# FatimaSohailll/KLT-Feature-Tracker-Acceleration-GPUs

Hardware: AMD Instinct MI355X
Metric: frames/sec + pyramid Gpix/s @1080p 5000 feats, 1/2/4/8 MI355X (higher is better)
Workload: dtype f32; 1 GPU; 1920x1080, 5000 features, sequential KLTTrackFeatures pass + KLTStoreFeatureList per frame, 2361 frames per GPU (BASELINE config 3; config 5 at N>1); device-resident: frames in HBM before timing, features and table stay on the device (the API-inclusive figure is the `api` key); chunk=64, chunk_requested=64, resolution=1920x1080, features=5000, frames=2361, parallelism=single GPU, reduction=exact

## Files before the change

include/klt_hip.h:

```cpp
#ifndef KLT_HIP_H
#define KLT_HIP_H

#include <stddef.h>

#ifdef __cplusplus
extern "C" {
#endif

#define KLT_HIP_MAX_TAPS 71
#define KLT_HIP_MAX_LEVELS 8
#define KLT_HIP_MAX_SLOTS 4

#define KLT_HIP_EXACT 0
#define KLT_HIP_FAST 1

typedef struct {
  int width;
  float k[KLT_HIP_MAX_TAPS];
} klt_hip_taps;

typedef struct {
  int ncols, nrows;
  int nlevels;
  int subsampling;
// ... 43 lines not shown
void klt_hip_ctx_destroy(klt_hip_ctx *ctx);
int klt_hip_ctx_reset(klt_hip_ctx *ctx);
int klt_hip_ctx_device(klt_hip_ctx *ctx);
int klt_hip_current_device(void);
const char *klt_hip_last_error(klt_hip_ctx *ctx);
const char *klt_hip_track_kernel(klt_hip_ctx *ctx);
int klt_hip_set_stream(klt_hip_ctx *ctx, void *stream);
void *klt_hip_get_stream(klt_hip_ctx *ctx);
int klt_hip_sync(klt_hip_ctx *ctx);
int klt_hip_device_count(void);

int klt_hip_upload_frame(klt_hip_ctx *ctx, int buf, const unsigned char *host, int ncols,
                         int nrows);
int klt_hip_build_pyramid(klt_hip_ctx *ctx, int slot, const klt_hip_pyr_desc *desc,
                          const unsigned char *frame, long pitch, int buf);

#define KLT_HIP_FRAME_GRAY8 0
#define KLT_HIP_FRAME_RGB8 1
#define KLT_HIP_FRAME_BGR8 2
#define KLT_HIP_FRAME_RGBA8 3
#define KLT_HIP_FRAME_BGRA8 4
int klt_hip_frame_bpp(int format);
int klt_hip_set_frame_format(klt_hip_ctx *ctx, int format);
int klt_hip_get_frame_format(klt_hip_ctx *ctx);
int klt_hip_gray_host(int format, const unsigned char *src, long pitch, int ncols, int nrows,
                      unsigned char *dst, long dst_pitch);
int klt_hip_to_gray(klt_hip_ctx *ctx, int format, const unsigned char *dev_src, long pitch, long stride,
                    int nframes, int ncols, int nrows, unsigned char *dev_dst, long dst_pitch, long dst_stride);
int klt_hip_set_path(klt_hip_ctx *ctx, int force_generic);
int klt_hip_set_track_order(klt_hip_ctx *ctx, int input_order);
int klt_hip_set_track_impl(klt_hip_ctx *ctx, int impl);
int klt_hip_set_track_merge(klt_hip_ctx *ctx, int on);
int klt_hip_set_lazy_grad(klt_hip_ctx *ctx, int on);
#define KLT_HIP_FB_REJECTED (-6)
int klt_hip_set_fb(klt_hip_ctx *ctx, int on, float max_dist);
int klt_hip_get_fb(klt_hip_ctx *ctx, int *on, float *max_dist);
int klt_hip_set_fb_table(klt_hip_ctx *ctx, float *dev_err, long stride);
int klt_hip_set_predict(klt_hip_ctx *ctx, int on, float *dev_vx, float *dev_vy);
int klt_hip_get_predict(klt_hip_ctx *ctx, int *on, float **dev_vx, float **dev_vy);
int klt_hip_set_predict_table(klt_hip_ctx *ctx, float *dev_tab_vx, float *dev_tab_vy, long stride);
#define KLT_HIP_MASKED (-7)
#define KLT_HIP_MASK_SELECT 1
#define KLT_HIP_MASK_TRACK 2
int klt_hip_set_mask(klt_hip_ctx *ctx, const unsigned char *dev_mask, long pitch, int flags);
int klt_hip_get_mask(klt_hip_ctx *ctx, const unsigned char **dev_mask, long *pitch, int *flags);
int klt_hip_set_track_prio(klt_hip_ctx *ctx, int on);
int klt_hip_set_track_count(klt_hip_ctx *ctx, int on);
int klt_hip_get_track_count(klt_hip_ctx *ctx, unsigned long long *solves, unsigned long long *passes,
                            int reset);
int klt_hip_set_track_patch(klt_hip_ctx *ctx, int on);
int klt_hip_set_prof(klt_hip_ctx *ctx, void *dev);
int klt_hip_set_host_threads(klt_hip_ctx *ctx, int workers);
int klt_hip_get_host_threads(klt_hip_ctx *ctx);
int klt_hip_register_host(klt_hip_ctx *ctx, const void *ptr, size_t bytes);
int klt_hip_unregister_host(klt_hip_ctx *ctx, const void *ptr);
int klt_hip_set_bank_budget(klt_hip_ctx *ctx, size_t bytes);
size_t klt_hip_get_bank_budget(klt_hip_ctx *ctx);
int klt_hip_frames_chunk(klt_hip_ctx *ctx);
size_t klt_hip_ctx_footprint(klt_hip_ctx *ctx);
int klt_hip_set_frames_overlap(klt_hip_ctx *ctx, int overlap);
int klt_hip_set_frames_tail(klt_hip_ctx *ctx, int waves_left);
int klt_hip_tail_threshold(unsigned base, unsigned launched, unsigned waves_left, unsigned *threshold);
int klt_hip_set_wave_times(klt_hip_ctx *ctx, void *dev);
int klt_hip_order_slot(int n, int xcd_per, int n_live, int rank, int lost, int *slot);
int klt_hip_band_order_probe(klt_hip_ctx *ctx, const float *y, const int *val, int n, int nrows, int *perm_out);
int klt_hip_fused_path(klt_hip_ctx *ctx, const klt_hip_pyr_desc *desc);
// ... 134 lines not shown
```

klt-feature-tracker-acceleration-gpus_amd/csrc/klt_dev.h:

```cpp
#pragma once

#include <hip/hip_runtime.h>
#include <stdint.h>

#include <string>

#include "klt_hip.h"

namespace kltdev {

constexpr int kWave = 64;
constexpr int kBlock = 256;

constexpr int kTracked = 0, kNotFound = -1, kSmallDet = -2, kMaxIter = -3, kOOB = -4, kLargeResidue = -5;

__host__ __device__ __forceinline__ int clampi(int v, int lo, int hi) { return v < lo ? lo : (v > hi ? hi : v); }

struct RTaps {
  int w;
  float k[KLT_HIP_MAX_TAPS];
};

inline RTaps reverse_taps(const klt_hip_taps &t) {
  RTaps r;
// ... 127 lines not shown
  const float *ai, *agx, *agy;
  const float *bi, *bgx, *bgy;
  int aw, ah, bw, bh;
  const float *xp, *yp;
  const float *x, *y;
  int *v;
  float *xo, *yo;
  float *aff;
  int *state;
  float *store;
  int n;
  AffParams p;
};

struct TrkAffArgs {
  AffParams p;
  float *aff;
  int *state;
  float *store;
  int fresh;
  int lds_wave;
  float *tab_aff;
  int *tab_state;
  long stride;
};
#ifndef KLT_AFF_CH
#define KLT_AFF_CH 64
#endif
constexpr int kAffChunk = KLT_AFF_CH;

hipError_t launch_pyr_l0(hipStream_t st, const uint8_t *src, int pitch, long stride, int W, int H, const DefTaps &T,
                         int vec_u8, int vec_out, float *img, float *gx, float *gy, float *hs, int W1, int do_hs,
                         long fs0, long fsh, int F, int ty0, int ty1, int py0 = 0, int py1 = 1 << 30, int il = 0,
                         int fmt = KLT_HIP_FRAME_GRAY8);
hipError_t launch_pyr_l1(hipStream_t st, const float *hs, int W1, int H, int H1, const DefTaps &T, int vec,
                         float *img1, float *gx1, float *gy1, long fsh, long fs1, int F, int ty0, int ty1, int il = 0,
                         int thin = 0);
constexpr int kL1ThinRows = 8;
hipError_t launch_u8_to_f32(hipStream_t st, const uint8_t *src, long pitch, int W, int H, float *out);
hipError_t launch_px_to_f32(hipStream_t st, const uint8_t *src, long pitch, int W, int H, int fmt, float *out);
hipError_t launch_to_gray(hipStream_t st, int fmt, const uint8_t *src, long pitch, long stride, int n, int W, int H,
                          uint8_t *dst, long dpitch, long dstride);
hipError_t launch_rows(hipStream_t st, const float *in, int W, int H, const RTaps &t, float *out);
hipError_t launch_cols(hipStream_t st, const float *in, int W, int H, const RTaps &t, float *out);
hipError_t launch_subsample(hipStream_t st, const float *in, int W, int ss, float *out, int W1, int H1);
hipError_t launch_min_eigen(hipStream_t st, const float *gx, const float *gy, int W, int ps, int bx, int by, int step,
                            int nx, int ny, int hw, int hh, int *out, const char **name = nullptr);
struct GradTaps {
  float g[2 * kRG + 1], d[2 * kRG + 1];
};
hipError_t launch_min_eigen_img(hipStream_t st, const float *img, int W, int H, const GradTaps &t, int bx, int by,
                                int step, int nx, int ny, int *out, const char **name = nullptr);
hipError_t launch_min_eigen_multi(hipStream_t st, const float *rec, long frame_stride, const EigMultiArgs &m, int W,
                                  int bx, int by, int step, int nx, int ny, int *maps, const char **name = nullptr);
hipError_t launch_synth(hipStream_t st, unsigned long long seed, int t0, int n, int W, int H, int row0, uint8_t *out,
                        long pitch, long fstride);
hipError_t launch_selftest_sqrt(const double *in, double *out, int n);
hipError_t launch_from_il(hipStream_t st, const float *il, float *img, float *gx, float *gy, long n);
hipError_t launch_to_il(hipStream_t st, const float *plane, float *il, int field, long n);
hipError_t launch_copy_words(hipStream_t st, const void *src, void *dst, long n);
hipError_t launch_selftest_div(const float *a, const float *b, float *out, int n);
hipError_t launch_selftest_solve2(const float *in, float step, float min_det, float *out, int *ok, int n);

hipError_t launch_track_frames(hipStream_t st, bool exact, bool li, bool patch, bool win7, int npx,
                               const TrkArgs &a, const TrkFramesArgs &b, float *x, float *y, int *v, int n,
                               const TrkFbArgs *fb = nullptr, const TrkAffArgs *af = nullptr);
size_t track_affine_lds_bytes(int mode);
// ... 60 lines not shown
```

klt-feature-tracker-acceleration-gpus_amd/csrc/pyramid.hip:

```cpp
#pragma clang fp contract(off)

#include <math.h>
#include <stdlib.h>

#include "klt_dev.h"
#include "klt_synth.h"

namespace kltdev {
namespace {

typedef float f2 __attribute__((ext_vector_type(2)));

typedef float f4 __attribute__((ext_vector_type(4)));

__device__ __forceinline__ f4 ld4(const float *p) { return *reinterpret_cast<const f4 *>(p); }
static_assert(kHsSlab == 16, "hs slab width");
__device__ __forceinline__ unsigned hs_at32(int y, int X, int H) {
  return ((unsigned)(X >> 4) * (unsigned)H + (unsigned)y) * 16u + (unsigned)(X & 15);
}
__device__ __forceinline__ void st4(float *p, f4 v) { *reinterpret_cast<f4 *>(p) = v; }
__device__ __forceinline__ void st4_out(float *p, f4 v) { __builtin_nontemporal_store(v, reinterpret_cast<f4 *>(p)); }
__device__ __forceinline__ void st2_out(float *p, f2 v) { __builtin_nontemporal_store(v, reinterpret_cast<f2 *>(p)); }
typedef float f3u __attribute__((ext_vector_type(3), aligned(4)));
__device__ __forceinline__ void st3_out(float *p, f3u v) { __builtin_nontemporal_store(v, reinterpret_cast<f3u *>(p)); }
// ... 551 lines not shown
template <bool IL, int TH_, bool IMG, int FMT>
__global__ __launch_bounds__(L0G<TH_>::NT) void k_pyr_l0_px(const uint8_t *__restrict__ src, int spitch, int W, int H,
                                                      DefTaps T, int vec_u8, float *__restrict__ img0,
                                                      float *__restrict__ gx0, float *__restrict__ gy0,
                                                      float *__restrict__ hs, int hsW, int do_hs, int vec_out,
                                                      long fs_src, long fs0, long fs_hs, int ty0, int tiles_x,
                                                      int tiles_y, int py0, int py1) {
  static_assert(FMT != KLT_HIP_FRAME_GRAY8, "gray frames take k_pyr_l0");
  using G = L0G<TH_, IMG ? 0 : kRG>;
  __shared__ __attribute__((aligned(16))) float lds[G::LDS];
  int bx, by;
  if (!xcd_tile(tiles_x, tiles_y, bx, by)) return;
#ifdef KLT_PYR_PROF
  const int tid = threadIdx.x;
  PYR_STAMP(0)
#endif
  const int C0 = bx * G::TW, R0 = (by + ty0) * G::TH;
  src += blockIdx.z * fs_src;
  img0 += blockIdx.z * fs0;
  gx0 += blockIdx.z * fs0;
  gy0 += blockIdx.z * fs0;
  hs += blockIdx.z * fs_hs;
  const bool cols_in = C0 >= 12 && C0 + 84 <= W, rows_in = R0 >= 5 && R0 + G::TH + 7 <= H;
  const bool interior = vec_u8 && vec_out && (hsW * G::SS == W) && (hsW % 2 == 0) && cols_in && rows_in;
  const bool planes = by + ty0 >= py0 && by + ty0 < py1;
  if (interior)
    pyr_l0_tile<true, IL, TH_, IMG, FMT>(lds, src, spitch, W, H, T, vec_u8, img0, gx0, gy0, hs, hsW, do_hs, vec_out, C0,
                                         R0, threadIdx.x, planes, true, true);
  else
    pyr_l0_tile<false, IL, TH_, IMG, FMT>(lds, src, spitch, W, H, T, vec_u8, img0, gx0, gy0, hs, hsW, do_hs, vec_out, C0,
                                          R0, threadIdx.x, planes, cols_in, rows_in);
}

template <int TH_>
struct L1G {
  static constexpr int RG = kRG, RP = kRP, SS = kSS, TW = geom::L1_TW, TH = TH_, NT = 256;
  static constexpr int JW = 40;
  static constexpr int JH = TH + 2 * RG;
  static constexpr int HR = SS * (JH - 1) + 2 * RP + 1;
  static constexpr int LDS_H = HR * JW, LDS_J = JH * JW, LDS_X = JH * TW;
  static constexpr int LDS = LDS_H + LDS_J;
  static_assert(2 * LDS_X + TH * 3 * TW <= LDS_H, "tx/ty and the interleaved output tile reuse the hs region");
};
static_assert(L1G<geom::L1_TH>::HR == geom::L1_HR, "geometry");
constexpr int kL1ThinTH = 8;

template <bool IL, int TH_>
__global__ __launch_bounds__(256) void k_pyr_l1(const float *__restrict__ hs, int W1, int H, int H1,
                                                DefTaps T, int vec, float *__restrict__ img1,
                                                float *__restrict__ gx1, float *__restrict__ gy1,
                                                long fs_hs, long fs1, int ty0, int tiles_x, int tiles_y) {
  using G = L1G<TH_>;
  constexpr int RG = G::RG, RP = G::RP, SS = G::SS, TW = G::TW, TH = G::TH, NT = G::NT, JW = G::JW, JH = G::JH,
                HR = G::HR, LDS_H = G::LDS_H, LDS_X = G::LDS_X, LDS = G::LDS;
  hs += blockIdx.z * fs_hs;
  img1 += blockIdx.z * fs1;
  gx1 += blockIdx.z * fs1;
  gy1 += blockIdx.z * fs1;
  __shared__ __attribute__((aligned(16))) float lds[LDS];
  float *hl = lds;
  float *im = lds + LDS_H;
  float *tx = lds;
  float *ty = lds + LDS_X;
  float *stg = lds + 2 * LDS_X;

  int bx, by;
// ... 485 lines not shown
    const float acc = lane == kSumGxx   ? S[0]
                      : lane == kSumGxy ? S[1]
                      : lane == kSumGyy ? S[2]
                      : lane == kSumEx  ? S[3]
                      : lane == kSumEy  ? S[4]
                                        : __int_as_float(0x7fc00000 + lane);
    float dx = 0.0f, dy = 0.0f, d = 0.0f, du = 0.0f;
    const float det1 = solve_det(S[0], S[1], S[2]);
    const float det2 = solve_det(lane_of(acc, kSumGxx), lane_of(acc, kSumGxy), lane_of(acc, kSumGyy));
    const int k1 = !(det1 < min_det), k2 = !(det2 < min_det), k3 = k1;
    if (k1) solve1(S, step, det1, dx, dy);
    if (k2) d = solve2(acc, lane_of(acc, kSumGxy), step, det2);
    if (k3) du = solve2u(S, lane == 0, step, det1);
    const float r[6] = {dx, dy, lane_of(d, 0), lane_of(d, 1), lane_of(du, 0), lane_of(du, 1)};
    if (lane == 0) {
#pragma unroll
      for (int k = 0; k < 6; ++k) out[6 * (long)i + k] = r[k];
      ok[i] = k1 | (k2 << 1) | (k3 << 2);
    }
  }
}

}

constexpr int kL0WideMinRows = 2000;
bool l0_wide() {
  static const bool on = [] {
    const char *v = getenv("KLT_L0_WIDE");
    return !(v && *v && atoi(v) == 0);
  }();
  return on;
}

namespace {
template <int FMT>
hipError_t launch_pyr_l0_px(hipStream_t st, const uint8_t *src, int pitch, long stride, int W, int H, const DefTaps &T,
                            int vec_u8, int vec_out, float *img, float *gx, float *gy, float *hs, int W1, int do_hs,
                            long fs0, long fsh, int F, int ty0, int ty1, int py0, int py1, int il) {
  const int tx = (W + l0::TW - 1) / l0::TW;
  const int nty = (H + l0::G32::TH - 1) / l0::G32::TH;
  if (l0_wide() && H >= kL0WideMinRows && ty0 == 0 && ty1 == nty && py0 == 0 && py1 >= nty) {
    using G = L0G<64>;
    const int ty = (H + G::TH - 1) / G::TH;
    const dim3 grid(xcd_grid(tx * ty), 1, F);
    if (il == kLayoutImg)
      hipLaunchKernelGGL((k_pyr_l0_px<false, 64, true, FMT>), grid, dim3(G::NT), 0, st, src, pitch, W, H, T, vec_u8, img,
                         gx, gy, hs, W1, do_hs, vec_out, stride, fs0, fsh, 0, tx, ty, 0, ty);
    else if (il)
      hipLaunchKernelGGL((k_pyr_l0_px<true, 64, false, FMT>), grid, dim3(G::NT), 0, st, src, pitch, W, H, T, vec_u8, img,
                         gx, gy, hs, W1, do_hs, vec_out, stride, fs0, fsh, 0, tx, ty, 0, ty);
    else
      hipLaunchKernelGGL((k_pyr_l0_px<false, 64, false, FMT>), grid, dim3(G::NT), 0, st, src, pitch, W, H, T, vec_u8,
                         img, gx, gy, hs, W1, do_hs, vec_out, stride, fs0, fsh, 0, tx, ty, 0, ty);
    return hipGetLastError();
  }
  using G = l0::G32;
  const dim3 grid(xcd_grid(tx * (ty1 - ty0)), 1, F);
  if (il == kLayoutImg)
    hipLaunchKernelGGL((k_pyr_l0_px<false, 32, true, FMT>), grid, dim3(G::NT), 0, st, src, pitch, W, H, T, vec_u8, img,
                       gx, gy, hs, W1, do_hs, vec_out, stride, fs0, fsh, ty0, tx, ty1 - ty0, py0, py1);
  else if (il)
    hipLaunchKernelGGL((k_pyr_l0_px<true, 32, false, FMT>), grid, dim3(G::NT), 0, st, src, pitch, W, H, T, vec_u8, img,
                       gx, gy, hs, W1, do_hs, vec_out, stride, fs0, fsh, ty0, tx, ty1 - ty0, py0, py1);
  else
    hipLaunchKernelGGL((k_pyr_l0_px<false, 32, false, FMT>), grid, dim3(G::NT), 0, st, src, pitch, W, H, T, vec_u8, img,
                       gx, gy, hs, W1, do_hs, vec_out, stride, fs0, fsh, ty0, tx, ty1 - ty0, py0, py1);
  return hipGetLastError();
}
}

hipError_t launch_pyr_l0(hipStream_t st, const uint8_t *src, int pitch, long stride, int W, int H, const DefTaps &T,
                         int vec_u8, int vec_out, float *img, float *gx, float *gy, float *hs, int W1, int do_hs,
                         long fs0, long fsh, int F, int ty0, int ty1, int py0, int py1, int il, int fmt) {
  const int tx = (W + l0::TW - 1) / l0::TW;
  if (F <= 0 || ty1 <= ty0) return hipSuccess;
  switch (fmt) {
    case KLT_HIP_FRAME_GRAY8: break;
#define KLT_L0_PX(f)                                                                                               \
  case f:                                                                                                          \
    return launch_pyr_l0_px<f>(st, src, pitch, stride, W, H, T, vec_u8, vec_out, img, gx, gy, hs, W1, do_hs, fs0, \
                               fsh, F, ty0, ty1, py0, py1, il);
      KLT_L0_PX(KLT_HIP_FRAME_RGB8)
      KLT_L0_PX(KLT_HIP_FRAME_BGR8)
      KLT_L0_PX(KLT_HIP_FRAME_RGBA8)
      KLT_L0_PX(KLT_HIP_FRAME_BGRA8)
#undef KLT_L0_PX
    default: return hipErrorInvalidValue;
  }
#ifdef KLT_EXP_NOHS
  do_hs = 0;
#endif
  const int nty = (H + l0::G32::TH - 1) / l0::G32::TH;
  if (l0_wide() && H >= kL0WideMinRows && ty0 == 0 && ty1 == nty && py0 == 0 && py1 >= nty) {
    using G = L0G<64>;
    const int ty = (H + G::TH - 1) / G::TH;
    if (il == kLayoutImg)
      hipLaunchKernelGGL((k_pyr_l0<false, 64, true>), dim3(xcd_grid(tx * ty), 1, F), dim3(G::NT), 0, st, src, pitch, W,
                         H, T, vec_u8, img, gx, gy, hs, W1, do_hs, vec_out, stride, fs0, fsh, 0, tx, ty, 0, ty);
    else if (il)
      hipLaunchKernelGGL((k_pyr_l0<true, 64>), dim3(xcd_grid(tx * ty), 1, F), dim3(G::NT), 0, st, src, pitch, W, H, T,
                         vec_u8, img, gx, gy, hs, W1, do_hs, vec_out, stride, fs0, fsh, 0, tx, ty, 0, ty);
    else
      hipLaunchKernelGGL((k_pyr_l0<false, 64>), dim3(xcd_grid(tx * ty), 1, F), dim3(G::NT), 0, st, src, pitch, W, H,
                         T, vec_u8, img, gx, gy, hs, W1, do_hs, vec_out, stride, fs0, fsh, 0, tx, ty, 0, ty);
    return hipGetLastError();
  }
  using G = l0::G32;
  if (il == kLayoutImg)
    hipLaunchKernelGGL((k_pyr_l0<false, 32, true>), dim3(xcd_grid(tx * (ty1 - ty0)), 1, F), dim3(G::NT), 0, st, src,
                       pitch, W, H, T, vec_u8, img, gx, gy, hs, W1, do_hs, vec_out, stride, fs0, fsh, ty0, tx, ty1 - ty0,
                       py0, py1);
  else if (il)
    hipLaunchKernelGGL((k_pyr_l0<true, 32>), dim3(xcd_grid(tx * (ty1 - ty0)), 1, F), dim3(G::NT), 0, st, src, pitch, W,
                       H, T, vec_u8, img, gx, gy, hs, W1, do_hs, vec_out, stride, fs0, fsh, ty0, tx, ty1 - ty0, py0, py1);
  else
    hipLaunchKernelGGL((k_pyr_l0<false, 32>), dim3(xcd_grid(tx * (ty1 - ty0)), 1, F), dim3(G::NT), 0, st, src, pitch,
                       W, H, T, vec_u8, img, gx, gy, hs, W1, do_hs, vec_out, stride, fs0, fsh, ty0, tx, ty1 - ty0, py0,
                       py1);
  return hipGetLastError();
}

hipError_t launch_pyr_l1(hipStream_t st, const float *hs, int W1, int H, int H1, const DefTaps &T, int vec,
                         float *img1, float *gx1, float *gy1, long fsh, long fs1, int F, int ty0, int ty1, int il,
                         int thin) {
  const int tx = (W1 + geom::L1_TW - 1) / geom::L1_TW;
// ... 190 lines not shown
```

klt-feature-tracker-acceleration-gpus_amd/csrc/runtime.h:

```cpp
#pragma once

#include <sys/resource.h>
#include <math.h>
#include <stdarg.h>
#include <stdint.h>
#include <stdio.h>
#include <stdlib.h>
#include <string.h>

#include <algorithm>
#include <set>
#include <string>
#include <vector>

#include "host_pool.h"
#include "klt_dev.h"
#include "klt_hip.h"

#define KLT_API extern "C" __attribute__((visibility("default")))

#ifndef KLT_LAZY_GRAD_DEFAULT
#define KLT_LAZY_GRAD_DEFAULT 1
#endif

// ... 101 lines not shown
  bool caller_pending = false;
  Slot slot[KLT_HIP_MAX_SLOTS + 2];
  uint8_t *d_u8[2] = {nullptr, nullptr};
  uint8_t *h_u8[2] = {nullptr, nullptr};
  hipEvent_t u8_done[2] = {nullptr, nullptr};
  size_t u8_cap = 0;
  int u8_w[2] = {0, 0}, u8_h[2] = {0, 0};
  float *d_hs = nullptr;
  size_t hs_cap = 0;
  float *d_tmp[2] = {nullptr, nullptr};
  size_t tmp_cap[2] = {0, 0};
  float *d_fx = nullptr, *d_fy = nullptr;
  int *d_fv = nullptr;
  float *d_feat = nullptr, *h_feat = nullptr;
  int feat_mode = 2;
  size_t f_cap = 0;
  int *d_eig = nullptr;
  size_t eig_cap = 0;
  SelEngine *sel = nullptr;
  std::vector<std::pair<const unsigned char *, size_t>> registered;
  float *d_aff_store = nullptr;
  size_t aff_store_cap = 0;
  int aff_S = 0;
  float *d_aff = nullptr, *d_xp = nullptr, *d_yp = nullptr, *d_astage = nullptr;
  size_t aff_cap = 0, xp_cap = 0, yp_cap = 0, astage_cap = 0;
  int *d_astate = nullptr, *d_aidx = nullptr;
  size_t astate_cap = 0, aidx_cap = 0;
  std::string err;
  int force_generic = 0;
  int frame_format = KLT_HIP_FRAME_GRAY8;
  int track_order = 0;
  int track_patch = 1;
  int track_merge = 1;
  int lazy_grad = KLT_LAZY_GRAD_DEFAULT;
  RTaps lazy_gg, lazy_gd;
  int track_prio = 1;
  float *pl_scr[2][KLT_HIP_MAX_LEVELS] = {};
  size_t pl_cap[2][KLT_HIP_MAX_LEVELS] = {};
  int track_impl = 0;
  const char *track_kernel = nullptr;
  int fb_on = 0;
  float fb_dist = 0.0f;
  float *fb_tab = nullptr;
  long fb_stride = 0;
  int pred_on = 0;
  float *pred_vx = nullptr, *pred_vy = nullptr;
  float *pred_tvx = nullptr, *pred_tvy = nullptr;
  long pred_stride = 0;
  float *d_pred = nullptr;
  size_t pred_cap = 0;
  const unsigned char *mask = nullptr;
  long mask_pitch = 0;
  int mask_flags = 0;
  int aff_on = 0;
  AffParams aff_p{};
  float *aff_dev = nullptr;
  int *aff_state_dev = nullptr;
  float *aff_tab = nullptr;
  int *aff_stab = nullptr;
  long aff_tab_stride = 0;
  int aff_fresh = 1, aff_depth = 0;
  int rep_on = 0;
  klt_hip_replace_desc rep{};
  long rep_frames = 0, rep_runs = 0, rep_filled = 0;
  std::vector<unsigned char> rep_changed;
  int *d_rep_map = nullptr;
// ... 269 lines not shown
```

klt-feature-tracker-acceleration-gpus_amd/csrc/runtime.hip:

```cpp
#include "runtime.h"

int kltdev::ctx_fail(klt_hip_ctx *c, const char *fmt, ...) {
  char buf[512];
  va_list ap;
  va_start(ap, fmt);
  vsnprintf(buf, sizeof buf, fmt, ap);
  va_end(ap);
  if (c) c->err = buf;
  return -1;
}

namespace {
hipError_t make_pstream(klt_hip_ctx *c) {
  static const bool low = [] {
    const char *v = getenv("KLT_PSTREAM_PRIO");
    return v && strcmp(v, "low") == 0;
  }();
  if (!low) return hipStreamCreateWithFlags(&c->pstream, hipStreamNonBlocking);
  int least = 0, greatest = 0;
  const hipError_t e = hipDeviceGetStreamPriorityRange(&least, &greatest);
  if (e != hipSuccess) return e;
  return hipStreamCreateWithPriority(&c->pstream, hipStreamNonBlocking, least);
}
}
// ... 221 lines not shown
  for (hipStream_t st : {c->own, c->pstream, c->cstream, c->dstream})
    if (st) HIPCHK(c, hipStreamSynchronize(st));
  if (klt_hip_ctx_footprint(c) > kKeepBytes) {
    free_banks(c);
    hipFree(c->d_ring);
    hipFree(c->d_rows);
    c->d_ring = nullptr;
    c->d_rows = nullptr;
    c->ring_cap = c->drows_cap = 0;
    if (c->h_stage) hipHostFree(c->h_stage);
    if (c->h_rows) hipHostFree(c->h_rows);
    c->h_stage = nullptr;
    c->h_rows = nullptr;
    c->stage_cap = c->hrows_cap = 0;
  }
  if (c->copy_threads != default_host_threads()) {
    delete c->pool;
    c->pool = nullptr;
    c->copy_threads = default_host_threads();
  }
  c->feat_mode = 2;
  for (auto &r : c->registered) (void)hipHostUnregister(const_cast<unsigned char *>(r.first));
  c->registered.clear();
  if (c->sel) sel_engine_set_threshold(c->sel, sel_default_threshold());
  c->bank_budget = 0;
  c->chunk_used = 0;
  c->stream = c->own;
  c->force_generic = 0;
  c->frame_format = KLT_HIP_FRAME_GRAY8;
  c->track_order = 0;
  c->track_patch = 1;
  c->track_merge = 1;
  c->lazy_grad = KLT_LAZY_GRAD_DEFAULT;
  c->track_prio = 1;
  c->track_impl = 0;
  c->track_kernel = nullptr;
  c->fb_on = 0;
  c->fb_dist = 0.0f;
  c->mask = nullptr;
  c->mask_pitch = 0;
  c->mask_flags = 0;
  c->fb_tab = nullptr;
  c->fb_stride = 0;
  c->pred_on = 0;
  c->pred_vx = c->pred_vy = nullptr;
  c->pred_tvx = c->pred_tvy = nullptr;
  c->pred_stride = 0;
  c->aff_on = 0;
  c->aff_dev = nullptr;
  c->aff_state_dev = nullptr;
  c->aff_tab = nullptr;
  c->aff_stab = nullptr;
  c->aff_tab_stride = 0;
  c->aff_fresh = 1;
  c->aff_depth = 0;
  c->rep_on = 0;
  c->rep_frames = c->rep_runs = c->rep_filled = 0;
  c->rep_changed.clear();
  c->eig_kernel = nullptr;
  c->frames_sched = kSchedOne;
  c->tail_left = kTailLeftDefault;
  c->wave_t = nullptr;
  c->ahead_ready = 0;
  c->prof = nullptr;
  if (forget_kept(c)) return -1;
  c->timing = false;
// ... 217 lines not shown

KLT_API int klt_hip_set_frames_tail(klt_hip_ctx *c, int waves_left) {
  if (!c) return fail(c, "set_frames_tail: null context");
  if (waves_left < 0) return fail(c, "set_frames_tail: %d waves left", waves_left);
  c->tail_left = waves_left;
  return 0;
}

KLT_API int klt_hip_tail_threshold(unsigned base, unsigned launched, unsigned waves_left, unsigned *threshold) {
  if (launched == 0 || launched <= waves_left) return 0;
  if (threshold) *threshold = base + (launched - waves_left);
  return 1;
}

KLT_API int klt_hip_set_wave_times(klt_hip_ctx *c, void *dev) {
  if (!c) return fail(c, "set_wave_times: null context");
  c->wave_t = (unsigned long long *)dev;
  return 0;
}

KLT_API int klt_hip_set_track_patch(klt_hip_ctx *c, int on) {
  if (!c) return fail(c, "set_track_patch: null context");
  c->track_patch = on ? 1 : 0;
  return 0;
}


KLT_API int klt_hip_set_lazy_grad(klt_hip_ctx *c, int on) {
  if (!c) return fail(c, "set_lazy_grad: null context");
  c->lazy_grad = on ? 1 : 0;
  return 0;
}

KLT_API int klt_hip_set_track_merge(klt_hip_ctx *c, int on) {
  if (!c) return fail(c, "set_track_merge: null context");
  c->track_merge = on ? 1 : 0;
  return 0;
}

KLT_API int klt_hip_set_track_prio(klt_hip_ctx *c, int on) {
  if (!c) return fail(c, "set_track_prio: null context");
  c->track_prio = on ? 1 : 0;
  return 0;
}

KLT_API int klt_hip_set_track_impl(klt_hip_ctx *c, int impl) {
  if (!c || impl < 0 || impl > 1) return fail(c, "set_track_impl: 0 (default kernel) or 1 (generic)");
  c->track_impl = impl;
  return 0;
}

KLT_API int klt_hip_set_fb(klt_hip_ctx *c, int on, float max_dist) {
  if (!c) return fail(c, "set_fb: null context");
  if (!(max_dist >= 0.0f) || !isfinite(max_dist))
    return fail(c, "set_fb: max_dist %g must be finite and >= 0", (double)max_dist);
  c->fb_on = on ? 1 : 0;
  c->fb_dist = max_dist;
  return 0;
}

KLT_API int klt_hip_get_fb(klt_hip_ctx *c, int *on, float *max_dist) {
  if (!c) return fail(c, "get_fb: null context");
  if (on) *on = c->fb_on;
  if (max_dist) *max_dist = c->fb_dist;
  return 0;
}
// ... 351 lines not shown
```

klt-feature-tracker-acceleration-gpus_amd/csrc/runtime_pyr.hip:

```cpp
#include "runtime.h"

bool fused_ok(const klt_hip_pyr_desc *d) {
  return d->smooth_input && d->smooth.width == 2 * kRS + 1 && d->grad_gauss.width == 2 * kRG + 1 &&
         d->grad_deriv.width == 2 * kRG + 1 && d->grad_deriv.k[kRG] == 0.0f && kDC == kRG &&
         (d->nlevels == 1 || (d->nlevels == 2 && d->subsampling == kSS && d->pyr.width == 2 * kRP + 1));
}

int ensure_slot(klt_hip_ctx *c, int s, const klt_hip_pyr_desc *d) {
  Slot &S = c->slot[s];
  int w = d->ncols, h = d->nrows;
  S.nlev = d->nlevels;
  S.ss = d->nlevels > 1 ? d->subsampling : 1;
  for (int l = 0; l < d->nlevels; ++l) {
    Level &L = S.lv[l];
    L.w = w;
    L.h = h;
    size_t n = (size_t)w * h;
    if (L.cap < n || !L.img) {
      if (L.img) hipFree(L.img);
      L.img = L.gx = L.gy = nullptr;
      const size_t m = n ? n : 1;
      HIPCHK(c, hipMalloc((void **)&L.img, 3 * m * sizeof(float)));
      L.gx = L.img + m;
      L.gy = L.img + 2 * m;
// ... 53 lines not shown
}

DefTaps default_taps(const klt_hip_pyr_desc *d) {
  DefTaps T;
  const RTaps s = reverse_taps(d->smooth), g = reverse_taps(d->grad_gauss);
  const RTaps dd = reverse_taps(d->grad_deriv), p = reverse_taps(d->pyr);
  for (int m = 0; m < 5; ++m) T.s[m] = s.k[m];
  for (int m = 0; m < 7; ++m) {
    T.g[m] = g.k[m];
    T.d[m] = dd.k[m];
  }
  for (int m = 0; m < 21; ++m) T.p[m] = d->nlevels > 1 ? p.k[m] : 0.0f;
  return T;
}

int launch_l0(klt_hip_ctx *c, hipStream_t st, const uint8_t *src, long pitch, long stride, int W, int H,
              const DefTaps &T, int vec_u8, int vec_out, float *img, float *gx, float *gy, float *hs, int W1,
              int do_hs, long fs0, long fsh, int F, int &r0, int &r1, int *p0 = nullptr, int *p1 = nullptr,
              int il = 0, int fmt = KLT_HIP_FRAME_GRAY8) {
  if (r1 <= r0 || F <= 0) return 0;
  const int TH = geom::L0_TH;
  const int nty = (H + TH - 1) / TH;
  const int ty0 = r0 / TH, ty1 = r1 >= H ? nty : clampi((r1 + TH - 1) / TH, ty0, nty);
  r0 = ty0 * TH;
  r1 = ty1 >= nty ? H : ty1 * TH;
  int py0 = ty0, py1 = ty1;
  if (p0 && p1) {
    py0 = clampi(*p0 / TH, ty0, ty1);
    py1 = *p1 >= H ? ty1 : clampi((*p1 + TH - 1) / TH, py0, ty1);
    *p0 = py0 * TH;
    *p1 = py1 >= nty ? H : py1 * TH;
  }
  return launched(c, "k_pyr_l0", launch_pyr_l0(st, src, (int)pitch, stride, W, H, T, vec_u8, vec_out, img, gx, gy,
                                               hs, W1, do_hs, fs0, fsh, F, ty0, ty1, py0, py1, il, fmt));
}

bool l1_thin() {
  static const bool on = [] {
    const char *v = getenv("KLT_L1_THIN");
    return !(v && *v && atoi(v) == 0);
  }();
  return on;
}

int build_fused(klt_hip_ctx *c, int s, const klt_hip_pyr_desc *d, const uint8_t *src, long pitch,
                hipStream_t st, int fmt) {
  Slot &S = c->slot[s];
  const int W = d->ncols, H = d->nrows;
  const DefTaps T = default_taps(d);
  const bool two = d->nlevels == 2;
  const int W1 = two ? S.lv[1].w : 0, H1 = two ? S.lv[1].h : 0;
  for (int l = 0; l < d->nlevels; ++l) S.lv[l].il = 1;
  if (two && grow(c, &c->d_hs, &c->hs_cap, (size_t)hs_size(W1 > 0 ? W1 : 1, H))) return -1;
  if ((long)W * H == 0) return 0;
  const int vec_u8 = vec_u8_ok(src, pitch, 0L, W);
  const int vec_out = (W % 4 == 0) ? 1 : 0;
  {
    TimedScope ts(c, T_L0, st);
    int r0 = 0, r1 = H;
    if (launch_l0(c, st, src, pitch, 0L, W, H, T, vec_u8, vec_out, S.lv[0].img, S.lv[0].gx, S.lv[0].gy, c->d_hs,
                  W1, (two && W1 > 0) ? 1 : 0, 0L, 0L, 1, r0, r1, nullptr, nullptr, 1, fmt))
      return -1;
  }
  if (two && (long)W1 * H1 > 0) {
    TimedScope ts(c, T_L1, st);
    const int vec = (W1 % 4 == 0 && W1 >= 8) ? 1 : 0;
    const int thin = l1_thin() ? 1 : 0, th = thin ? kL1ThinRows : geom::L1_TH;
// ... 342 lines not shown
```

klt-feature-tracker-acceleration-gpus_amd/device.py:

```python
from __future__ import annotations

import ctypes
import ctypes as C
import os

MAX_TAPS = 71
MAX_LEVELS = 8
EXACT, FAST = 0, 1
FB_REJECTED = -6
MAX_SEQUENCES = 64
FRAME_GRAY8, FRAME_RGB8, FRAME_BGR8, FRAME_RGBA8, FRAME_BGRA8 = range(5)


class Taps(C.Structure):
    _fields_ = [("width", C.c_int), ("k", C.c_float * MAX_TAPS)]


class PyrDesc(C.Structure):
    _fields_ = [("ncols", C.c_int), ("nrows", C.c_int), ("nlevels", C.c_int),
                ("subsampling", C.c_int), ("smooth_input", C.c_int), ("smooth", Taps),
                ("pyr", Taps), ("grad_gauss", Taps), ("grad_deriv", Taps)]


class TrackDesc(C.Structure):
# ... 40 lines not shown
                ("ms_pyr_l1", C.c_double), ("ms_track", C.c_double), ("ms_eigen", C.c_double),
                ("ms_generic", C.c_double), ("frames_pyr_l0", C.c_long), ("frames_pyr_l1", C.c_long),
                ("frames_track", C.c_long)]


V = C.c_void_p
FP = C.POINTER(C.c_float)
IP = C.POINTER(C.c_int)
DP = C.POINTER(C.c_double)

DEVICE_PROTOS = {
    "klt_hip_ctx_create": (V, [C.c_int]),
    "klt_hip_ctx_destroy": (None, [V]),
    "klt_hip_last_error": (C.c_char_p, [V]),
    "klt_hip_track_kernel": (C.c_char_p, [V]),
    "klt_hip_set_stream": (C.c_int, [V, V]),
    "klt_hip_get_stream": (V, [V]),
    "klt_hip_sync": (C.c_int, [V]),
    "klt_hip_device_count": (C.c_int, []),
    "klt_hip_current_device": (C.c_int, []),
    "klt_hip_upload_frame": (C.c_int, [V, C.c_int, V, C.c_int, C.c_int]),
    "klt_hip_build_pyramid": (C.c_int, [V, C.c_int, C.POINTER(PyrDesc), V, C.c_long, C.c_int]),
    "klt_hip_frame_bpp": (C.c_int, [C.c_int]),
    "klt_hip_set_frame_format": (C.c_int, [V, C.c_int]),
    "klt_hip_get_frame_format": (C.c_int, [V]),
    "klt_hip_gray_host": (C.c_int, [C.c_int, V, C.c_long, C.c_int, C.c_int, V, C.c_long]),
    "klt_hip_to_gray": (C.c_int, [V, C.c_int, V, C.c_long, C.c_long, C.c_int, C.c_int, C.c_int, V, C.c_long,
                                  C.c_long]),
    "klt_hip_pyramid_path": (C.c_int, [V, C.c_int]),
    "klt_hip_fused_path": (C.c_int, [V, C.POINTER(PyrDesc)]),
    "klt_hip_set_track_order": (C.c_int, [V, C.c_int]),
    "klt_hip_set_track_merge": (C.c_int, [V, C.c_int]),
    "klt_hip_set_lazy_grad": (C.c_int, [V, C.c_int]),
    "klt_hip_set_track_prio": (C.c_int, [V, C.c_int]),
    "klt_hip_set_track_impl": (C.c_int, [V, C.c_int]),
    "klt_hip_set_track_patch": (C.c_int, [V, C.c_int]),
    "klt_hip_set_fb": (C.c_int, [V, C.c_int, C.c_float]),
    "klt_hip_get_fb": (C.c_int, [V, IP, FP]),
    "klt_hip_set_fb_table": (C.c_int, [V, V, C.c_long]),
    "klt_hip_set_predict": (C.c_int, [V, C.c_int, V, V]),
    "klt_hip_get_predict": (C.c_int, [V, IP, C.POINTER(V), C.POINTER(V)]),
    "klt_hip_set_predict_table": (C.c_int, [V, V, V, C.c_long]),
    "klt_hip_set_mask": (C.c_int, [V, V, C.c_long, C.c_int]),
    "klt_hip_get_mask": (C.c_int, [V, C.POINTER(V), C.POINTER(C.c_long), IP]),
    "klt_hip_set_frames_affine": (C.c_int, [V, C.POINTER(AffineDesc), V, V]),
    "klt_hip_get_frames_affine": (C.c_int, [V, IP]),
    "klt_hip_set_affine_table": (C.c_int, [V, V, V, C.c_long]),
    "klt_hip_affine_state_put": (C.c_int, [V, FP, IP, C.c_int, C.POINTER(V), C.POINTER(V)]),
    "klt_hip_affine_state_get": (C.c_int, [V, FP, IP, C.c_int]),
    "klt_hip_affine_reserve": (C.c_int, [V, C.c_int, C.c_int, C.c_int]),
    "klt_hip_affine_put": (C.c_int, [V, IP, C.c_int, FP]),
    "klt_hip_affine_get": (C.c_int, [V, IP, C.c_int, FP]),
    "klt_hip_track_affine": (C.c_int, [V, C.c_int, C.c_int, C.POINTER(TrackDesc), C.POINTER(AffineDesc), FP, FP, IP,
                                       FP, IP, C.c_int]),
    "klt_hip_set_frames_replace": (C.c_int, [V, C.POINTER(ReplaceDesc)]),
    "klt_hip_get_frames_replace": (C.c_int, [V, IP, C.POINTER(C.c_long), C.POINTER(C.c_long), C.POINTER(C.c_long)]),
    "klt_hip_frames_replace_changed": (C.c_int, [V, V, C.c_int]),
    "klt_hip_min_eigen_plane": (C.c_int, [V, V, C.c_int, C.c_int, C.POINTER(SelectDesc), V]),
    "klt_hip_eigen_kernel": (C.c_char_p, [V]),
    "klt_hip_set_track_count": (C.c_int, [V, C.c_int]),
    "klt_hip_get_track_count": (C.c_int, [V, C.POINTER(C.c_ulonglong), C.POINTER(C.c_ulonglong), C.c_int]),
    "klt_hip_set_prof": (C.c_int, [V, V]),
    "klt_hip_set_frames_overlap": (C.c_int, [V, C.c_int]),
    "klt_hip_set_frames_tail": (C.c_int, [V, C.c_int]),
    "klt_hip_tail_threshold": (C.c_int, [C.c_uint, C.c_uint, C.c_uint, C.POINTER(C.c_uint)]),
    "klt_hip_set_wave_times": (C.c_int, [V, V]),
# ... 130 lines not shown
```

Baseline: 131,100 frames/s.

## Add column-strip streaming kernel for level-0 pyramid smoothing and subsample

```diff
diff --git a/include/klt_hip.h b/include/klt_hip.h
--- a/include/klt_hip.h
+++ b/include/klt_hip.h
@@ -99,6 +99,7 @@
 int klt_hip_set_track_impl(klt_hip_ctx *ctx, int impl);
 int klt_hip_set_track_merge(klt_hip_ctx *ctx, int on);
 int klt_hip_set_lazy_grad(klt_hip_ctx *ctx, int on);
+int klt_hip_set_l0_strip(klt_hip_ctx *ctx, int on);
 #define KLT_HIP_FB_REJECTED (-6)
 int klt_hip_set_fb(klt_hip_ctx *ctx, int on, float max_dist);
 int klt_hip_get_fb(klt_hip_ctx *ctx, int *on, float *max_dist);
diff --git a/klt-feature-tracker-acceleration-gpus_amd/csrc/klt_dev.h b/klt-feature-tracker-acceleration-gpus_amd/csrc/klt_dev.h
--- a/klt-feature-tracker-acceleration-gpus_amd/csrc/klt_dev.h
+++ b/klt-feature-tracker-acceleration-gpus_amd/csrc/klt_dev.h
@@ -183,7 +183,7 @@
 hipError_t launch_pyr_l0(hipStream_t st, const uint8_t *src, int pitch, long stride, int W, int H, const DefTaps &T,
                          int vec_u8, int vec_out, float *img, float *gx, float *gy, float *hs, int W1, int do_hs,
                          long fs0, long fsh, int F, int ty0, int ty1, int py0 = 0, int py1 = 1 << 30, int il = 0,
-                         int fmt = KLT_HIP_FRAME_GRAY8);
+                         int fmt = KLT_HIP_FRAME_GRAY8, int strips = 0);
 hipError_t launch_pyr_l1(hipStream_t st, const float *hs, int W1, int H, int H1, const DefTaps &T, int vec,
                          float *img1, float *gx1, float *gy1, long fsh, long fs1, int F, int ty0, int ty1, int il = 0,
                          int thin = 0);
diff --git a/klt-feature-tracker-acceleration-gpus_amd/csrc/pyramid.hip b/klt-feature-tracker-acceleration-gpus_amd/csrc/pyramid.hip
--- a/klt-feature-tracker-acceleration-gpus_amd/csrc/pyramid.hip
+++ b/klt-feature-tracker-acceleration-gpus_amd/csrc/pyramid.hip
@@ -607,6 +607,123 @@
                                           R0, threadIdx.x, planes, cols_in, rows_in);
 }
 
+namespace l0s {
+constexpr int SW = 192;
+constexpr int HALO = 32;
+constexpr int PITCH = 8 + 256 + 16;
+constexpr int kSeg = 108;
+constexpr int kRing = 10;
+constexpr int lcm(int a, int b) {
+  int x = a;
+  while (x % b) x += a;
+  return x;
+}
+}
+
+__device__ __forceinline__ uint32_t lane_left(uint32_t v) {
+  return (uint32_t)__builtin_amdgcn_update_dpp((int)v, (int)v, 0x138 , 0xF, 0xF, false);
+}
+__device__ __forceinline__ uint32_t lane_right(uint32_t v) {
+  return (uint32_t)__builtin_amdgcn_update_dpp((int)v, (int)v, 0x130 , 0xF, 0xF, false);
+}
+__device__ __forceinline__ void l0s_lds_sync() {
+  __builtin_amdgcn_fence(__ATOMIC_RELEASE, "wavefront");
+  __builtin_amdgcn_wave_barrier();
+  __builtin_amdgcn_fence(__ATOMIC_ACQUIRE, "wavefront");
+}
+
+template <int PF, bool EDGE>
+__device__ __forceinline__ void pyr_l0_strip(float *__restrict__ lds, const uint8_t *__restrict__ src, int spitch, int W,
+                                             int H, const DefTaps &T, float *__restrict__ img0,
+                                             float *__restrict__ hs, int S, int y0, int y1) {
+  constexpr int RS = kRS, RP = kRP, U = l0s::lcm(10, PF), PITCH = l0s::PITCH;
+  const int lane = threadIdx.x;
+  const int px = S - l0s::HALO + 4 * lane;
+  const uint8_t *col = src + clampi(px, 0, W - 4);
+  const bool stores = lane >= 8 && lane < 56 && px < W;
+  const int X = px >> 2;
+  bool okx[4], okc = true;
+#pragma unroll
+  for (int e = 0; e < 4; ++e) okx[e] = px + e >= RS && px + e < W - RS;
+  okc = px + 2 >= RP && px + 2 < W - RP;
+  float *wr = lds + 8 + 4 * lane;
+
+  uint32_t ring[PF];
+#pragma unroll
+  for (int k = 0; k < PF; ++k)
+    ring[k] = *reinterpret_cast<const uint32_t *>(col + (unsigned)(clampi(y0 - RS + k, 0, H - 1) * spitch));
+  f4 win[5];
+  int r = y0 - RS;
+  auto rows = [&](int RK, int WK) {
+    const uint32_t d = ring[RK];
+    ring[RK] = *reinterpret_cast<const uint32_t *>(col + (unsigned)(clampi(r + PF, 0, H - 1) * spitch));
+    const uint32_t dl = lane_left(d), dr = lane_right(d);
+    const float v[8] = {(float)((dl >> 16) & 0xFF), (float)(dl >> 24),          (float)(d & 0xFF),  (float)((d >> 8) & 0xFF),
+                        (float)((d >> 16) & 0xFF),  (float)(d >> 24),           (float)(dr & 0xFF), (float)((dr >> 8) & 0xFF)};
+    f4 a = mul4(v, T.s[0]);
+#pragma unroll
+    for (int m = 1; m < 5; ++m) mac4(a, v + m, T.s[m]);
+    if (EDGE) {
+#pragma unroll
+      for (int e = 0; e < 4; ++e)
+        if (!okx[e]) a[e] = 0.0f;
+    }
+    win[WK] = a;
+  };
+#pragma unroll
+  for (int k = 0; k < 4; ++k) {
+    rows(k % PF, k);
+    ++r;
+  }
+  const int rend = y1 + RS;
+  while (r < rend) {
+#pragma unroll
+    for (int k = 0; k < U; ++k) {
+      if (r >= rend) continue;
+      rows((k + 4) % PF, (k + 4) % 5);
+      const int y = r - RS;
+      f4 acc = mul4(reinterpret_cast<const float *>(&win[(k + 0) % 5]), T.s[0]);
+#pragma unroll
+      for (int m = 1; m < 5; ++m) mac4(acc, reinterpret_cast<const float *>(&win[(k + m) % 5]), T.s[m]);
+      if (EDGE && !(y >= RS && y < H - RS)) acc = f4{0.0f, 0.0f, 0.0f, 0.0f};
+      if (stores) st4_out(img0 + (unsigned)(y * W + px), acc);
+      float *b = wr + (k & 1) * PITCH;
+      st4(b, acc);
+      l0s_lds_sync();
+      const f4 q0 = ld4(b - 8), q1 = ld4(b - 4), q3 = ld4(b + 4), q4 = ld4(b + 8);
+      const float q5 = b[12];
+      const float w[21] = {q0.x,  q0.y,  q0.z,  q0.w, q1.x, q1.y, q1.z, q1.w, acc.x, acc.y, acc.z,
+                           acc.w, q3.x,  q3.y,  q3.z, q3.w, q4.x, q4.y, q4.z, q4.w,  q5};
+      float h = w[0] * T.p[0];
+#pragma unroll
+      for (int m = 1; m < 21; ++m) {
+        float t = w[m] * T.p[m];
+        asm("" : "+v"(t));
+        h += t;
+      }
+      if (EDGE && !okc) h = 0.0f;
+      if (stores) hs[hs_at32(y, X, H)] = h;
+      ++r;
+    }
+  }
+}
+
+template <int PF>
+__global__ __launch_bounds__(64) void k_pyr_l0s(const uint8_t *__restrict__ src, int spitch, int W, int H, DefTaps T,
+                                                   float *__restrict__ img0, float *__restrict__ hs, long fs_src,
+                                                   long fs0, long fs_hs, int nstrips, int nseg, int seg) {
+  __shared__ __attribute__((aligned(16))) float lds[2 * l0s::PITCH];
+  int sx, sg;
+  if (!xcd_tile(nstrips, nseg, sx, sg)) return;
+  const int S = sx * l0s::SW, y0 = sg * seg, y1 = min(y0 + seg, H);
+  src += blockIdx.z * fs_src;
+  img0 += blockIdx.z * fs0;
+  hs += blockIdx.z * fs_hs;
+  const bool inside = S >= l0s::SW && S + 206 <= W && y0 >= kRS && y1 <= H - kRS;
+  if (inside) pyr_l0_strip<PF, false>(lds, src, spitch, W, H, T, img0, hs, S, y0, y1);
+  else pyr_l0_strip<PF, true>(lds, src, spitch, W, H, T, img0, hs, S, y0, y1);
+}
+
 template <int TH_>
 struct L1G {
   static constexpr int RG = kRG, RP = kRP, SS = kSS, TW = geom::L1_TW, TH = TH_, NT = 256;
@@ -1158,6 +1275,14 @@
   return on;
 }
 
+bool l0_strips(int ctx_choice) {
+  static const int env = [] {
+    const char *v = getenv("KLT_L0_STRIP");
+    return (v && *v) ? (atoi(v) != 0 ? 1 : 0) : -1;
+  }();
+  return env >= 0 ? env != 0 : ctx_choice != 0;
+}
+
 namespace {
 template <int FMT>
 hipError_t launch_pyr_l0_px(hipStream_t st, const uint8_t *src, int pitch, long stride, int W, int H, const DefTaps &T,
@@ -1197,7 +1322,7 @@
 
 hipError_t launch_pyr_l0(hipStream_t st, const uint8_t *src, int pitch, long stride, int W, int H, const DefTaps &T,
                          int vec_u8, int vec_out, float *img, float *gx, float *gy, float *hs, int W1, int do_hs,
-                         long fs0, long fsh, int F, int ty0, int ty1, int py0, int py1, int il, int fmt) {
+                         long fs0, long fsh, int F, int ty0, int ty1, int py0, int py1, int il, int fmt, int strips) {
   const int tx = (W + l0::TW - 1) / l0::TW;
   if (F <= 0 || ty1 <= ty0) return hipSuccess;
   switch (fmt) {
@@ -1217,6 +1342,13 @@
   do_hs = 0;
 #endif
   const int nty = (H + l0::G32::TH - 1) / l0::G32::TH;
+  if (l0_strips(strips) && il == kLayoutImg && do_hs && ty0 == 0 && ty1 == nty && py0 == 0 && py1 >= nty && vec_u8 &&
+      vec_out && W1 * l0::SS == W && W1 % 2 == 0) {
+    const int ns = (W + l0s::SW - 1) / l0s::SW, nseg = (H + l0s::kSeg - 1) / l0s::kSeg;
+    hipLaunchKernelGGL(k_pyr_l0s<l0s::kRing>, dim3(xcd_grid(ns * nseg), 1, F), dim3(kWave), 0, st, src, pitch, W, H, T,
+                       img, hs, stride, fs0, fsh, ns, nseg, l0s::kSeg);
+    return hipGetLastError();
+  }
   if (l0_wide() && H >= kL0WideMinRows && ty0 == 0 && ty1 == nty && py0 == 0 && py1 >= nty) {
     using G = L0G<64>;
     const int ty = (H + G::TH - 1) / G::TH;
diff --git a/klt-feature-tracker-acceleration-gpus_amd/csrc/runtime.h b/klt-feature-tracker-acceleration-gpus_amd/csrc/runtime.h
--- a/klt-feature-tracker-acceleration-gpus_amd/csrc/runtime.h
+++ b/klt-feature-tracker-acceleration-gpus_amd/csrc/runtime.h
@@ -157,6 +157,7 @@
   int track_order = 0;
   int track_patch = 1;
   int track_merge = 1;
+  int l0_strip = 1;
   int lazy_grad = KLT_LAZY_GRAD_DEFAULT;
   RTaps lazy_gg, lazy_gd;
   int track_prio = 1;
diff --git a/klt-feature-tracker-acceleration-gpus_amd/csrc/runtime.hip b/klt-feature-tracker-acceleration-gpus_amd/csrc/runtime.hip
--- a/klt-feature-tracker-acceleration-gpus_amd/csrc/runtime.hip
+++ b/klt-feature-tracker-acceleration-gpus_amd/csrc/runtime.hip
@@ -277,6 +277,7 @@
   c->track_patch = 1;
   c->track_merge = 1;
   c->lazy_grad = KLT_LAZY_GRAD_DEFAULT;
+  c->l0_strip = 1;
   c->track_prio = 1;
   c->track_impl = 0;
   c->track_kernel = nullptr;
@@ -560,6 +561,12 @@
   return 0;
 }
 
+KLT_API int klt_hip_set_l0_strip(klt_hip_ctx *c, int on) {
+  if (!c) return fail(c, "set_l0_strip: null context");
+  c->l0_strip = on ? 1 : 0;
+  return 0;
+}
+
 KLT_API int klt_hip_set_track_merge(klt_hip_ctx *c, int on) {
   if (!c) return fail(c, "set_track_merge: null context");
   c->track_merge = on ? 1 : 0;
diff --git a/klt-feature-tracker-acceleration-gpus_amd/csrc/runtime_pyr.hip b/klt-feature-tracker-acceleration-gpus_amd/csrc/runtime_pyr.hip
--- a/klt-feature-tracker-acceleration-gpus_amd/csrc/runtime_pyr.hip
+++ b/klt-feature-tracker-acceleration-gpus_amd/csrc/runtime_pyr.hip
@@ -109,7 +109,8 @@
     *p1 = py1 >= nty ? H : py1 * TH;
   }
   return launched(c, "k_pyr_l0", launch_pyr_l0(st, src, (int)pitch, stride, W, H, T, vec_u8, vec_out, img, gx, gy,
-                                               hs, W1, do_hs, fs0, fsh, F, ty0, ty1, py0, py1, il, fmt));
+                                               hs, W1, do_hs, fs0, fsh, F, ty0, ty1, py0, py1, il, fmt,
+                                               c->l0_strip));
 }
 
 bool l1_thin() {
diff --git a/klt-feature-tracker-acceleration-gpus_amd/device.py b/klt-feature-tracker-acceleration-gpus_amd/device.py
--- a/klt-feature-tracker-acceleration-gpus_amd/device.py
+++ b/klt-feature-tracker-acceleration-gpus_amd/device.py
@@ -96,6 +96,7 @@
     "klt_hip_set_track_order": (C.c_int, [V, C.c_int]),
     "klt_hip_set_track_merge": (C.c_int, [V, C.c_int]),
     "klt_hip_set_lazy_grad": (C.c_int, [V, C.c_int]),
+    "klt_hip_set_l0_strip": (C.c_int, [V, C.c_int]),
     "klt_hip_set_track_prio": (C.c_int, [V, C.c_int]),
     "klt_hip_set_track_impl": (C.c_int, [V, C.c_int]),
     "klt_hip_set_track_patch": (C.c_int, [V, C.c_int]),
```

New measurement: 135,500 frames/s, median of 6. +3.4%, better.
